# rmontanana/semcode

Measured on AMD Instinct MI355X. Metric: chunks/sec embed (256-tok) + top-k QPS over 10M x 768, higher is better.
Workload: dtype bf16; 1 GPU; encoder forward, 256 chunks x 256 tokens per GPU per step, BERT-base shape (12x768, 12 heads, FFN 3072), bf16 MFMA / f32 accumulate, random-init weights; global_batch=256, seq_len=256, parallelism=dp1 (replicated weights, no collective), device=AMD Radeon Graphics (gfx950:sramecc+:xnack-)

## Files before the change

### include/semcode_hip.h

```cpp
#ifndef SEMCODE_HIP_H
#define SEMCODE_HIP_H

#include <stddef.h>
#include <stdint.h>

#ifdef __cplusplus
extern "C" {
#endif

typedef int32_t sc_status;

enum {
    SC_OK = 0,
    SC_ERR_INVALID = -1,
    SC_ERR_HIP = -2,
    SC_ERR_STATE = -3,
    SC_ERR_UNSUPPORTED = -4,
    SC_ERR_NOMEM = -5
};

typedef enum { SC_METRIC_IP = 0, SC_METRIC_L2 = 1, SC_METRIC_COSINE = 2 } sc_metric;
typedef enum { SC_INDEX_FLAT = 0, SC_INDEX_IVF_FLAT = 1 } sc_index_kind;

typedef struct sc_runtime sc_runtime;
// ... 61 lines not shown
sc_status sc_tokenizer_create(const char* vocab_utf8, size_t nbytes, int32_t lowercase, sc_tokenizer** out);
sc_status sc_tokenizer_destroy(sc_tokenizer* tok);
sc_status sc_tokenizer_info(sc_tokenizer* tok, int32_t* vocab_size, int32_t* pad, int32_t* unk, int32_t* cls, int32_t* sep);
sc_status sc_tokenizer_encode(sc_tokenizer* tok, const char* bytes, const int64_t* offsets, int32_t n, int32_t max_tokens, int32_t S,
                              int32_t* ids, int32_t* lens, uint8_t* needs_fallback, int32_t threads);

sc_status sc_diag_gemm_bf16(sc_runtime* rt, int32_t epi, const float* A, const float* W, const float* bias, const float* R,
                            int32_t M, int32_t N, int32_t K, float* out);
sc_status sc_diag_gemm_bench(sc_runtime* rt, int32_t epi, int32_t M, int32_t N, int32_t K, int32_t iters, int32_t variant,
                             double* ms_per_launch);
sc_status sc_diag_gemm_trace(sc_runtime* rt, int32_t epi, int32_t M, int32_t N, int32_t K, uint64_t* out, int64_t cap_words);
sc_status sc_diag_gemm_i8(sc_runtime* rt, const int8_t* A, const int8_t* W, int32_t M, int32_t N, int32_t K, int32_t* out);
sc_status sc_diag_encoder_read(sc_encoder* enc, int32_t which, void* out, size_t nbytes);
sc_status sc_diag_set_option(const char* name, int32_t value);
sc_status sc_diag_rope(sc_runtime* rt, float* qk, int32_t rows, int32_t S, int32_t heads, float theta);
sc_status sc_diag_swiglu(sc_runtime* rt, const float* h, int32_t rows, int32_t F, float* out);
sc_status sc_diag_attention(sc_runtime* rt, const float* qkv, const int32_t* lens, int32_t B, int32_t S, int32_t heads, float* out);

sc_status sc_diag_fold_ln(sc_runtime* rt, const float* W, const float* gamma, const float* beta, const float* bias, int32_t N, int32_t K,
                          float* Wf, float* c1, float* c2);
sc_status sc_diag_gemm_lna(sc_runtime* rt, int32_t epi, int32_t flags, const float* A, const float* Wf, const float* c1, const float* c2,
                           const float* stats_in, float eps, int32_t M, int32_t N, int32_t K, int32_t rope_S, float rope_theta,
                           int32_t rope_ncols, float* C, float* fin);
sc_status sc_diag_gemm_resln(sc_runtime* rt, int32_t flags, const float* A, const float* W, const float* bias, const float* gam, const float* R,
                             const float* fin, float eps, int32_t M, int32_t N, int32_t K, float* C, float* stats_out);
sc_status sc_diag_attention_ex(sc_runtime* rt, const float* qkv, const int32_t* lens, int32_t B, int32_t S, int32_t heads, int32_t blocked_rows,
                               const float* slopes, float* out);
sc_status sc_diag_attention_packed(sc_runtime* rt, const float* qkv, const int32_t* starts, const int32_t* lens, int32_t B, int32_t heads,
                                   int32_t blocked_rows, const float* slopes, float* out);
sc_status sc_diag_layernorm(sc_runtime* rt, const float* x, int32_t tokens, int32_t H, const float* gamma, const float* beta, float eps, float* out);
sc_status sc_diag_mean_pool(sc_runtime* rt, const float* x, const int32_t* lens, int32_t B, int32_t S, int32_t H, int32_t normalize, float* out);
sc_status sc_diag_mean_pool_ln(sc_runtime* rt, const float* y, const float* stats, int32_t slots, int32_t tokens_pad, const float* gamma,
                               const float* beta, float eps, const int32_t* lens, int32_t B, int32_t S, int32_t H, float* out);
sc_status sc_diag_geglu(sc_runtime* rt, const float* h, int32_t rows, int32_t F, float* out);
sc_status sc_diag_embed(sc_runtime* rt, int32_t ln, const int32_t* ids, int32_t tokens, int32_t S, int32_t H, int32_t vocab, int32_t max_pos,
                        const float* wemb, const float* pemb, const float* temb, const float* gamma, const float* beta, float eps,
                        int32_t tokens_pad, int32_t slots, float* rows, float* stats);


sc_status sc_index_create(sc_runtime* rt, int32_t dim, sc_metric metric, sc_index_kind kind,
                          int32_t nlist, int64_t row_base, sc_index** out);
sc_status sc_index_destroy(sc_index* ix);
sc_status sc_index_info(sc_index* ix, int64_t* rows, int32_t* dim, int32_t* ld);
sc_status sc_index_reserve(sc_index* ix, int64_t rows);
sc_status sc_index_add(sc_index* ix, const float* vecs, int64_t n);
sc_status sc_index_overwrite(sc_index* ix, const float* vecs, const int64_t* rows, int64_t n);
// ... 80 lines not shown
```

### semcode_amd/_native.py

```python
from __future__ import annotations

import ctypes as C
import sys
import threading
from pathlib import Path

import numpy as np

LIB_PATH = Path(__file__).resolve().parent / "_lib" / "libsemcode_hip.so"

METRICS = {"IP": 0, "L2": 1, "COSINE": 2}
KINDS = {"FLAT": 0, "IVF_FLAT": 1}


class ScError(RuntimeError):

    def __init__(self, status: int, message: str):
        super().__init__(f"libsemcode_hip error {status}: {message}")
        self.status = status


class _Cfg(C.Structure):
    _fields_ = [("device", C.c_int32), ("stream", C.c_void_p), ("flags", C.c_int32)]

# ... 30 lines not shown
    "sc_encoder_embed_ids": (C.c_int32, [C.c_void_p, C.c_void_p, C.c_void_p, C.c_int32, C.c_int32, C.c_void_p]),
    "sc_encoder_embed_ids_dev": (C.c_int32, [C.c_void_p, C.c_void_p, C.c_void_p, C.c_int32, C.c_int32, C.c_void_p]),
    "sc_encoder_embed_ids_into": (C.c_int32, [C.c_void_p, C.c_void_p, C.c_void_p, C.c_int32, C.c_int32, C.c_void_p, C.c_void_p, C.c_void_p]),
    "sc_encoder_embed_ids_into_async": (C.c_int32, [C.c_void_p, C.c_void_p, C.c_void_p, C.c_int32, C.c_int32, C.c_void_p, C.c_void_p]),
    "sc_encoder_wait": (C.c_int32, [C.c_void_p]),
    "sc_encoder_packed_rows": (C.c_int32, [C.c_void_p, C.c_void_p, C.c_int32, C.POINTER(C.c_int64)]),
    "sc_encoder_embed_packed": (C.c_int32, [C.c_void_p, C.c_void_p, C.c_void_p, C.c_int32, C.c_void_p]),
    "sc_encoder_embed_packed_into": (C.c_int32, [C.c_void_p, C.c_void_p, C.c_void_p, C.c_int32, C.c_void_p, C.c_void_p, C.c_void_p]),
    "sc_encoder_embed_packed_into_async": (C.c_int32, [C.c_void_p, C.c_void_p, C.c_void_p, C.c_int32, C.c_void_p, C.c_void_p]),
    "sc_tokenizer_create": (C.c_int32, [C.c_char_p, C.c_size_t, C.c_int32, C.POINTER(C.c_void_p)]),
    "sc_tokenizer_destroy": (C.c_int32, [C.c_void_p]),
    "sc_tokenizer_info": (C.c_int32, [C.c_void_p] + [C.POINTER(C.c_int32)] * 5),
    "sc_tokenizer_encode": (C.c_int32, [C.c_void_p, C.c_char_p, C.c_void_p, C.c_int32, C.c_int32, C.c_int32, C.c_void_p, C.c_void_p, C.c_void_p, C.c_int32]),
    "sc_diag_gemm_bf16": (C.c_int32, [C.c_void_p, C.c_int32, C.c_void_p, C.c_void_p, C.c_void_p, C.c_void_p, C.c_int32, C.c_int32, C.c_int32, C.c_void_p]),
    "sc_diag_gemm_bench": (C.c_int32, [C.c_void_p, C.c_int32, C.c_int32, C.c_int32, C.c_int32, C.c_int32, C.c_int32, C.POINTER(C.c_double)]),
    "sc_diag_gemm_trace": (C.c_int32, [C.c_void_p, C.c_int32, C.c_int32, C.c_int32, C.c_int32, C.c_void_p, C.c_int64]),
    "sc_diag_set_option": (C.c_int32, [C.c_char_p, C.c_int32]),
    "sc_diag_gemm_i8": (C.c_int32, [C.c_void_p, C.c_void_p, C.c_void_p, C.c_int32, C.c_int32, C.c_int32, C.c_void_p]),
    "sc_diag_encoder_read": (C.c_int32, [C.c_void_p, C.c_int32, C.c_void_p, C.c_size_t]),
    "sc_diag_attention": (C.c_int32, [C.c_void_p, C.c_void_p, C.c_void_p, C.c_int32, C.c_int32, C.c_int32, C.c_void_p]),
    "sc_diag_rope": (C.c_int32, [C.c_void_p, C.c_void_p, C.c_int32, C.c_int32, C.c_int32, C.c_float]),
    "sc_diag_swiglu": (C.c_int32, [C.c_void_p, C.c_void_p, C.c_int32, C.c_int32, C.c_void_p]),
    "sc_diag_fold_ln": (C.c_int32, [C.c_void_p] * 5 + [C.c_int32, C.c_int32] + [C.c_void_p] * 3),
    "sc_diag_gemm_lna": (C.c_int32, [C.c_void_p, C.c_int32, C.c_int32] + [C.c_void_p] * 5 + [C.c_float, C.c_int32, C.c_int32, C.c_int32, C.c_int32,
                                     C.c_float, C.c_int32, C.c_void_p, C.c_void_p]),
    "sc_diag_gemm_resln": (C.c_int32, [C.c_void_p, C.c_int32] + [C.c_void_p] * 6 + [C.c_float, C.c_int32, C.c_int32, C.c_int32, C.c_void_p, C.c_void_p]),
    "sc_diag_attention_ex": (C.c_int32, [C.c_void_p, C.c_void_p, C.c_void_p, C.c_int32, C.c_int32, C.c_int32, C.c_int32, C.c_void_p, C.c_void_p]),
    "sc_diag_attention_packed": (C.c_int32, [C.c_void_p, C.c_void_p, C.c_void_p, C.c_void_p, C.c_int32, C.c_int32, C.c_int32, C.c_void_p, C.c_void_p]),
    "sc_diag_layernorm": (C.c_int32, [C.c_void_p, C.c_void_p, C.c_int32, C.c_int32, C.c_void_p, C.c_void_p, C.c_float, C.c_void_p]),
    "sc_diag_mean_pool": (C.c_int32, [C.c_void_p, C.c_void_p, C.c_void_p, C.c_int32, C.c_int32, C.c_int32, C.c_int32, C.c_void_p]),
    "sc_diag_mean_pool_ln": (C.c_int32, [C.c_void_p, C.c_void_p, C.c_void_p, C.c_int32, C.c_int32, C.c_void_p, C.c_void_p, C.c_float, C.c_void_p,
                                         C.c_int32, C.c_int32, C.c_int32, C.c_void_p]),
    "sc_diag_geglu": (C.c_int32, [C.c_void_p, C.c_void_p, C.c_int32, C.c_int32, C.c_void_p]),
    "sc_diag_embed": (C.c_int32, [C.c_void_p, C.c_int32, C.c_void_p, C.c_int32, C.c_int32, C.c_int32, C.c_int32, C.c_int32] + [C.c_void_p] * 5 +
                                 [C.c_float, C.c_int32, C.c_int32, C.c_void_p, C.c_void_p]),
    "sc_index_create": (C.c_int32, [C.c_void_p, C.c_int32, C.c_int32, C.c_int32, C.c_int32, C.c_int64, C.POINTER(C.c_void_p)]),
    "sc_index_destroy": (C.c_int32, [C.c_void_p]),
    "sc_index_info": (C.c_int32, [C.c_void_p, C.POINTER(C.c_int64), C.POINTER(C.c_int32), C.POINTER(C.c_int32)]),
    "sc_index_reserve": (C.c_int32, [C.c_void_p, C.c_int64]),
    "sc_index_add": (C.c_int32, [C.c_void_p, C.c_void_p, C.c_int64]),
    "sc_index_overwrite": (C.c_int32, [C.c_void_p, C.c_void_p, C.c_void_p, C.c_int64]),
    "sc_index_put_rows": (C.c_int32, [C.c_void_p, C.c_void_p, C.c_void_p, C.c_int64]),
    "sc_index_put_rows_dev": (C.c_int32, [C.c_void_p, C.c_void_p, C.c_void_p, C.c_int64]),
    "sc_index_delete_rows": (C.c_int32, [C.c_void_p, C.c_void_p, C.c_int64]),
    "sc_index_last_delete_stats": (C.c_int32, [C.c_void_p, C.POINTER(C.c_int64), C.POINTER(C.c_int64), C.POINTER(C.c_int32), C.POINTER(C.c_int32)]),
    "sc_index_get_rows": (C.c_int32, [C.c_void_p, C.c_int64, C.c_int64, C.c_void_p]),
# ... 736 lines not shown

def diag_fold_ln(rt: Runtime, W, gamma, beta, bias=None):
    W, gamma, beta = _f32(W), _f32(gamma), _f32(beta)
    bias = None if bias is None else _f32(bias)
    N, K = W.shape
    Wf, c1, c2 = np.empty((N, K), np.float32), np.empty(N, np.float32), np.empty(N, np.float32)
    _check(lib().sc_diag_fold_ln(rt.handle, _ptr(W), _ptr(gamma), _ptr(beta), _ptr(bias), N, K, _ptr(Wf), _ptr(c1), _ptr(c2)))
    return Wf, c1, c2


def diag_gemm_lna(rt: Runtime, epi: int, A, Wf, c1, c2, stats_in, eps: float, blocked: bool = False, rope_S: int = 0, rope_theta: float = 0.0,
                  rope_ncols: int = 0):
    A, Wf, c1, c2, stats_in = _f32(A), _f32(Wf), _f32(c1), _f32(c2), _f32(stats_in)
    M, K = A.shape
    N = Wf.shape[0]
    if stats_in.shape != (K // 256, M, 2) or Wf.shape != (N, K) or c1.shape != (N,) or c2.shape != (N,):
        raise ValueError("diag_gemm_lna: shapes")
    Cc, fin = np.empty((M, N), np.float32), np.empty((M, 2), np.float32)
    _check(lib().sc_diag_gemm_lna(rt.handle, epi, 1 if blocked else 0, _ptr(A), _ptr(Wf), _ptr(c1), _ptr(c2), _ptr(stats_in), float(eps), M, N, K,
                                  int(rope_S), float(rope_theta), int(rope_ncols), _ptr(Cc), _ptr(fin)))
    return (unblock64(Cc, M, N) if blocked else Cc), fin


def diag_gemm_resln(rt: Runtime, A, W, bias, gam, R, fin, eps: float, a_blocked: bool = False):
    A, W, bias, gam, R, fin = _f32(A), _f32(W), _f32(bias), _f32(gam), _f32(R), _f32(fin)
    M, K = A.shape
    N = W.shape[0]
    if W.shape != (N, K) or R.shape != (M, N) or fin.shape != (M, 2) or bias.shape != (N,) or gam.shape != (N,):
        raise ValueError("diag_gemm_resln: shapes")
    Ad = block64(A) if a_blocked else A
    Cc, st = np.empty((M, N), np.float32), np.empty((N // 256, M, 2), np.float32)
    _check(lib().sc_diag_gemm_resln(rt.handle, 1 if a_blocked else 0, _ptr(Ad), _ptr(W), _ptr(bias), _ptr(gam), _ptr(R), _ptr(fin), float(eps), M, N, K,
                                    _ptr(Cc), _ptr(st)))
    return Cc, st


def diag_attention_ex(rt: Runtime, qkv, lens, B: int, S: int, heads: int, blocked_rows: int = 0, slopes=None) -> np.ndarray:
    qkv = _f32(qkv)
    lens = np.ascontiguousarray(lens, np.int32)
    H = heads * 64
    if blocked_rows:
        pad = np.zeros((blocked_rows, 3 * H), np.float32)
        pad[: B * S] = qkv
        qkv = block64(pad)
    sl = None if slopes is None else _f32(slopes)
    out = np.empty((B * S, H), np.float32)
# ... 87 lines not shown
```

### semcode_amd/csrc/encoder_ops.h

```cpp
#pragma once
#include <vector>

#include "sc_common.h"

enum { EPI_BIAS = 0, EPI_BIAS_GELU = 1, EPI_BIAS_RES = 2, EPI_LNA_BIAS = 3, EPI_LNA_GELU = 4, EPI_RESLN_STATS = 5, EPI_LNA_BIAS_ROPE = 6 };

bool sc_gemm_bf16_supported(int M, int N, int K);
void sc_launch_gemm_bf16(int epi, const void* A, int lda, const void* W, int ldw, const float* bias, const void* R, int ldr, void* C,
                         int ldc, int M, int N, int K, hipStream_t s, void* splitk_scratch = nullptr, size_t splitk_scratch_bytes = 0);
int sc_gemm_splitk_factor(int M, int N, int K, int cus);
bool sc_gemm_ln_supported(int M, int N, int K);
void sc_launch_gemm_bf16_ln(int epi, const void* A, int lda, const void* W, int ldw, const float* bias, const void* R, int ldr, void* C, int ldc, int M,
                            int N, int K, hipStream_t s, const float* c1, const float* stats_in, float* fin, const float* gam, float* stats_out, float eps,
                            const float* rope_cos = nullptr, const float* rope_sin = nullptr, int rope_S = 0, int rope_ncols = 0);
void sc_launch_gemm_i8_diag(const void* A, const void* W, void* C, int M, int N, int K, hipStream_t s);
void sc_gemm_set_debug(int v);
void sc_gemm_set_order(int v);
void sc_gemm_set_pp(int v);
void sc_gemm_set_nt(int v);
void sc_gemm_set_trace(unsigned long long* dev);
void sc_gemm_force_tile128(bool on);

void sc_launch_embed_ln(const int32_t* ids, int tokens, int S, int H, int vocab, int max_pos, const float* wemb, const float* pemb,
                        const float* temb, const float* g, const float* b, float eps, void* out, hipStream_t s);
void sc_launch_layernorm(const void* in, int tokens, int H, const float* g, const float* b, float eps, void* out, hipStream_t s);
bool sc_attention_supported(int S, int H, int heads);
void sc_launch_attention(const void* qkv, const int32_t* lens, int B, int S, int H, const float* slopes, void* ctx, hipStream_t s, int blocked = 0);
void sc_launch_geglu(const void* h, int64_t tokens, int F, void* out, hipStream_t s);
void sc_launch_swiglu(const void* h, int64_t tokens, int F, void* out, hipStream_t s);
void sc_launch_rope_qk(void* qkv, int64_t M, int nblocks, int S, const float* cos_t, const float* sin_t, hipStream_t s);
void sc_launch_embed_raw(const int32_t* ids, int tokens, int tokens_pad, int S, int H, int vocab, int max_pos, const float* wemb, const float* pemb,
                         const float* temb, void* out, float* stats, int slots, hipStream_t s);
void sc_launch_fold_ln_weights(const float* W, const float* gamma, const float* beta, const float* bias, int N, int K, void* Wf, float* c1, float* c2,
                               hipStream_t s);
void sc_launch_add_vectors(const float* a, const float* b, float* out, int n, hipStream_t s);
void sc_launch_mean_pool_ln(const void* y, const float* stats, int slots, int tokens_pad, const float* gamma, const float* beta, float eps,
                            const int32_t* lens, int B, int S, int H, float* out, hipStream_t s);
void sc_launch_mean_pool(const void* x, const int32_t* lens, int B, int S, int H, int normalize, float* out, hipStream_t s);
void sc_launch_f32_to_bf16(const float* in, void* out, int64_t n, hipStream_t s);
void sc_launch_synth_scaled(float* out, int64_t n, uint64_t seed, float scale, float offset, hipStream_t s);
void sc_launch_bf16_to_f32(const void* in, float* out, int64_t n, hipStream_t s);

// ... 16 lines not shown
```

### semcode_amd/csrc/gemm_bf16.hip

```cpp
#include <algorithm>
#include <cstdlib>

#include "encoder_ops.h"
#include "gemm_tile.h"

#ifndef SC_GEMM_PP_DEFAULT
#define SC_GEMM_PP_DEFAULT 4
#endif


struct GemmArgs {
    const bf16_t* A;
    const bf16_t* W;
    const float* bias;
    const bf16_t* R;
    bf16_t* C;
    int M, N, K, lda, ldw, ldr, ldc;
    int tiles_n;
    int ntiles;
    int order;
    int splitk;
    float* partial;
    unsigned long long* trace;
    int nt;
    int cblock;
    int ablock;
    const float* c1;
    const float* stats_in;
    int stat_slots;
    float* fin;
    const float* gam;
    float* stats_out;
    float ln_eps;
    const float* rope_cos;
    const float* rope_sin;
    int rope_smask, rope_ncols;
};

static __device__ __forceinline__ size_t c_index(const GemmArgs& a, int64_t m, int n) {
    return a.cblock ? ((size_t)(n >> 6) * (size_t)a.M + (size_t)m) * 64 + (size_t)(n & 63) : (size_t)m * a.ldc + n;
}

template <int EPI>
__global__ __launch_bounds__(256) void gemm_bf16_kernel(GemmArgs a) {
// ... 182 lines not shown
        for (int ni = 0; ni < 4; ++ni) {
            f32x4 v = acc[ni][mi] + bias4[ni];
            if (EPI == EPI_BIAS_GELU) {
                const f32x2 g0 = gelu_erf_fast2(f32x2{v[0], v[1]}), g1 = gelu_erf_fast2(f32x2{v[2], v[3]});
                v = f32x4{g0[0], g0[1], g1[0], g1[1]};
            }
            if (EPI == EPI_BIAS_RES) {
                const u32x2 r2 = rr[mi][ni];
                v += f32x4{__builtin_bit_cast(float, r2[0] << 16), __builtin_bit_cast(float, r2[0] & 0xFFFF0000u),
                           __builtin_bit_cast(float, r2[1] << 16), __builtin_bit_cast(float, r2[1] & 0xFFFF0000u)};
            }
            *reinterpret_cast<u32x2*>(stg + fr * T_EPI_ROW + (ni * 16 + 4 * fq) * 2) = u32x2{pack_bf16x2(v[0], v[1]), pack_bf16x2(v[2], v[3])};
        }
#pragma unroll
        for (int j = 0; j < 2; ++j) {
            const u32x4 o = *reinterpret_cast<const u32x4*>(stg + (j * 8 + prow) * T_EPI_ROW + c8 * 2);
            bf16_t* dst = cp + (size_t)(mi * 16 + j * 8) * crs;
            if (a.nt) asm volatile("global_store_dwordx4 %0, %1, off nt" ::"v"(dst), "v"(o) : "memory");
            else *reinterpret_cast<u32x4*>(dst) = o;
        }
    }
}

template <int EPI>
static __device__ __forceinline__ void gemm256_epilogue_lna(const GemmArgs& a, int m0, int n0, char* smem, int w, int lane, f32x4 (&acc)[4][8]) {
    const int wm = w >> 2, wn = w & 3;
    int ln = lane;
    asm volatile("" : "+v"(ln));
    __builtin_amdgcn_sched_barrier(0);
    const int fr = ln & 15, fq = ln >> 4;
    const int prow = ln >> 3, c8 = (ln & 7) * 8;
    char* stg = smem + 4 * T_TILE_BYTES + w * (16 * T_EPI_ROW);
    typedef uint32_t u32x2 __attribute__((ext_vector_type(2)));
    typedef uint32_t u32x4 __attribute__((ext_vector_type(4)));
    typedef float f32x2_t __attribute__((ext_vector_type(2)));
    f32x4 c1v[4], c2v[4];
#pragma unroll
    for (int ni = 0; ni < 4; ++ni) {
        c1v[ni] = *reinterpret_cast<const f32x4*>(a.c1 + n0 + wn * 64 + ni * 16 + 4 * fq);
        c2v[ni] = *reinterpret_cast<const f32x4*>(a.bias + n0 + wn * 64 + ni * 16 + 4 * fq);
    }
    asm volatile("s_waitcnt vmcnt(0)" ::: "memory");
    char* slice = smem + w * 16384;
    {
        f32x4 sacc = {0.f, 0.f, 0.f, 0.f};
        for (int t = 0; t < a.stat_slots; ++t) sacc += *reinterpret_cast<const f32x4*>(slice + t * 1024 + ln * 16);
        const float inv_k = 1.0f / (float)a.K;
        const float mu0 = sacc[0] * inv_k, mu1 = sacc[2] * inv_k;
        const float rs0 = __builtin_amdgcn_rsqf(fmaxf(fmaf(-mu0, mu0, sacc[1] * inv_k), 0.f) + a.ln_eps);
        const float rs1 = __builtin_amdgcn_rsqf(fmaxf(fmaf(-mu1, mu1, sacc[3] * inv_k), 0.f) + a.ln_eps);
        const f32x4 fin4 = {mu0, rs0, mu1, rs1};
        *reinterpret_cast<f32x4*>(slice + ln * 16) = fin4;
        if (n0 == 0 && wn == 0) *reinterpret_cast<f32x4*>(a.fin + (size_t)(m0 + wm * 128) * 2 + ln * 4) = fin4;
    }
    const char* sl = slice + fr * 8;
    const size_t crs = a.cblock ? 64 : (size_t)a.ldc;
    bf16_t* cp = a.C + c_index(a, m0 + wm * 128 + prow, n0 + wn * 64) + c8;
#pragma unroll
    for (int mi = 0; mi < 8; ++mi) {
        const f32x2_t st = *reinterpret_cast<const f32x2_t*>(sl + mi * 128);
        const float mu = st[0], rs = st[1];
        f32x2 nrm = {-rs * mu, -rs * mu}, rs2 = {rs, rs};
        SC_OPAQUE_PAIR(nrm);
        SC_OPAQUE_PAIR(rs2);
#pragma unroll
        for (int ni = 0; ni < (EPI == EPI_LNA_BIAS_ROPE ? 0 : 4); ++ni) {
            const f32x2 d01 = __builtin_elementwise_fma(nrm, f32x2{c1v[ni][0], c1v[ni][1]}, f32x2{c2v[ni][0], c2v[ni][1]});
            const f32x2 d23 = __builtin_elementwise_fma(nrm, f32x2{c1v[ni][2], c1v[ni][3]}, f32x2{c2v[ni][2], c2v[ni][3]});
            const f32x2 v01 = __builtin_elementwise_fma(rs2, f32x2{acc[ni][mi][0], acc[ni][mi][1]}, d01);
            const f32x2 v23 = __builtin_elementwise_fma(rs2, f32x2{acc[ni][mi][2], acc[ni][mi][3]}, d23);
            f32x4 v = {v01[0], v01[1], v23[0], v23[1]};
            if (EPI == EPI_LNA_GELU) {
                const f32x2 g0 = gelu_erf_fast2(f32x2{v[0], v[1]}), g1 = gelu_erf_fast2(f32x2{v[2], v[3]});
                v = f32x4{g0[0], g0[1], g1[0], g1[1]};
            }
            *reinterpret_cast<u32x2*>(stg + fr * T_EPI_ROW + (ni * 16 + 4 * fq) * 2) = u32x2{pack_bf16x2(v[0], v[1]), pack_bf16x2(v[2], v[3])};
        }
        if constexpr (EPI == EPI_LNA_BIAS_ROPE) {
// ... 170 lines not shown
                                         ResLnCoopHook{ResidualCoopHook{a.R + (size_t)m0 * a.ldr + n0, a.ldr, w, lane, smem},
                                                       a.fin + (size_t)(m0 + (w >> 2) * 128) * 2}, a_kstep);
        else
            gemm256_mainloop_sel<PP, ML>(a, lda, m0, n0, smem, acc, w, lane,
                                         ResLnTailHook{ResidualTailHook{a.R + (size_t)m0 * a.ldr + n0, a.ldr, w, lane, smem},
                                                       a.fin + (size_t)(m0 + (w >> 2) * 128) * 2}, a_kstep);
    }
    else if (EPI == EPI_LNA_BIAS || EPI == EPI_LNA_GELU || EPI == EPI_LNA_BIAS_ROPE)
        gemm256_mainloop_sel<PP, ML>(a, lda, m0, n0, smem, acc, w, lane,
                                     LnaTailHook{a.stats_in + (size_t)(m0 + (w >> 2) * 128) * 2, (size_t)a.M * 2, a.stat_slots, w, lane, smem}, a_kstep);
    else
        gemm256_mainloop_sel<PP, ML>(a, lda, m0, n0, smem, acc, w, lane, NoTailHook{}, a_kstep);
    gemm256_stamp(a, blockIdx.x, 3);
    if (DBG & 4) {
        float sink = 0.f;
#pragma unroll
        for (int i = 0; i < 4; ++i)
#pragma unroll
            for (int j = 0; j < 8; ++j) sink += acc[i][j][0] + acc[i][j][3];
        if (sink == 12345.678f) a.C[0] = 1;
        return;
    }
    if (EPI == EPI_RESLN_STATS) gemm256_epilogue_resln<COOP>(a, m0, n0, smem, w, lane, acc);
    else if (EPI == EPI_LNA_BIAS || EPI == EPI_LNA_GELU || EPI == EPI_LNA_BIAS_ROPE) gemm256_epilogue_lna<EPI>(a, m0, n0, smem, w, lane, acc);
    else gemm256_epilogue<EPI, COOP && !(DBG & 31)>(a, m0, n0, smem, w, lane, acc);
    if (a.trace) {
        gemm256_stamp(a, blockIdx.x, 4);
        asm volatile("s_waitcnt vmcnt(0)" ::: "memory");
        gemm256_stamp(a, blockIdx.x, 5);
    }
}

__global__ __launch_bounds__(512) void gemm256_i8_diag_kernel(const int8_t* __restrict__ A, const int8_t* __restrict__ W, int32_t* __restrict__ C, int M, int N,
                                                               int K) {
    extern __shared__ __attribute__((aligned(16))) char smem[];
    const int lane = threadIdx.x & 63;
    const int w = __builtin_amdgcn_readfirstlane(threadIdx.x >> 6);
    const int tiles_n = N / T_BN;
    const int m0 = ((int)blockIdx.x / tiles_n) * T_BM, n0 = ((int)blockIdx.x % tiles_n) * T_BN;
    f32x4 acc[4][8];
#pragma unroll
    for (int i = 0; i < 4; ++i)
#pragma unroll
        for (int j = 0; j < 8; ++j) acc[i][j] = f32x4{0.f, 0.f, 0.f, 0.f};
    gemm_tile256_mainloop<0, NoTailHook, true>(reinterpret_cast<const bf16_t*>(A), K / 2, m0, reinterpret_cast<const bf16_t*>(W), K / 2, n0, K / 2, smem, acc, w, lane);
    int ln = lane;
    asm volatile("" : "+v"(ln));
    const int wm = w >> 2, wn = w & 3, fr = ln & 15, fq = ln >> 4;
    int32_t* out = C + (size_t)(m0 + wm * 128 + fr) * N + n0 + wn * 64 + 4 * fq;
#pragma unroll
    for (int mi = 0; mi < 8; ++mi)
#pragma unroll
// ... 62 lines not shown
    }
}

int sc_gemm_splitk_factor(int M, int N, int K, int cus) {
    if ((M % T_BM) || (N % T_BN) || M > 1024) return 1;
    const int tiles = (M / T_BM) * (N / T_BN), nk = K / G_BK;
    int best = 1;
    for (int d = 2; d <= nk; ++d)
        if (nk % d == 0 && nk / d >= 3 && tiles * d <= cus) best = d;
    return tiles * 2 <= cus ? best : 1;
}

static int g_gemm_pp = -1;
void sc_gemm_set_pp(int v) { g_gemm_pp = v; }
static int gemm_pp() {
    static const char* env = getenv("SC_GEMM_PP");
    return g_gemm_pp >= 0 ? g_gemm_pp : env ? atoi(env) : SC_GEMM_PP_DEFAULT;
}
static int g_gemm_nt = -1;
void sc_gemm_set_nt(int v) { g_gemm_nt = v < 0 ? -1 : (v ? 1 : 0); }
static int gemm_nt(int M, int N) {
    static const char* env_nt = getenv("SC_GEMM_NT");
    return g_gemm_nt >= 0 ? g_gemm_nt : env_nt ? atoi(env_nt) : ((size_t)M * (size_t)N * 2 >= ((size_t)64 << 20));
}
template <int EPI, int DBG, int PP>
static void launch256_pp(const GemmArgs& a, dim3 grid, dim3 block, hipStream_t s) {
    static ScDeviceOnce once;
    sc_device_once(once, [&] { hipFuncSetAttribute(reinterpret_cast<const void*>(gemm256_bf16_kernel<EPI, DBG, PP>), hipFuncAttributeMaxDynamicSharedMemorySize, (int)T_LDS_BYTES); });
    hipLaunchKernelGGL((gemm256_bf16_kernel<EPI, DBG, PP>), grid, block, T_LDS_BYTES, s, a);
}
template <int EPI, int DBG>
static void launch256(const GemmArgs& a, dim3 grid, dim3 block, hipStream_t s) {
    const int pp = a.K >= 2 * G_BK ? gemm_pp() : 0;
    if (pp == 0) return launch256_pp<EPI, DBG, 0>(a, grid, block, s);
    if constexpr (DBG == 4) {
        if (pp == 3) return launch256_pp<EPI, DBG, 3>(a, grid, block, s);
        if (pp == 5) return launch256_pp<EPI, DBG, 5>(a, grid, block, s);
    }
    launch256_pp<EPI, DBG, 4>(a, grid, block, s);
}
template <int DBG>
static void launch256_epi(int epi, const GemmArgs& a, dim3 grid, dim3 block, hipStream_t s) {
    if (epi == EPI_BIAS_GELU) launch256<EPI_BIAS_GELU, DBG>(a, grid, block, s);
    else if (epi == EPI_BIAS_RES) launch256<EPI_BIAS_RES, DBG>(a, grid, block, s);
    else launch256<EPI_BIAS, DBG>(a, grid, block, s);
}

bool sc_gemm_ln_supported(int M, int N, int K) { return M > 0 && (M % T_BM) == 0 && (N % T_BN) == 0 && (K % 256) == 0; }
void sc_launch_gemm_bf16_ln(int epi, const void* A, int lda, const void* W, int ldw, const float* bias, const void* R, int ldr, void* C, int ldc, int M,
                            int N, int K, hipStream_t s, const float* c1, const float* stats_in, float* fin, const float* gam, float* stats_out, float eps,
                            const float* rope_cos, const float* rope_sin, int rope_S, int rope_ncols) {
    GemmArgs a;
    a.rope_cos = rope_cos; a.rope_sin = rope_sin; a.rope_smask = rope_S - 1; a.rope_ncols = rope_ncols;
    a.A = (const bf16_t*)A; a.W = (const bf16_t*)W; a.bias = bias; a.R = (const bf16_t*)R; a.C = (bf16_t*)C;
    a.M = M; a.N = N; a.K = K; a.lda = lda; a.ldw = ldw; a.ldr = ldr; a.ldc = ldc;
    a.cblock = ldc == SC_LDC_BLOCKED64 ? 1 : 0;
    a.ablock = lda == SC_LDC_BLOCKED64 ? 1 : 0;
    static const char* env_order = getenv("SC_GEMM_ORDER");
    a.order = env_order ? atoi(env_order) : ((size_t)N * (size_t)K * 2 <= ((size_t)8 << 20) ? 0 : 16);
    a.trace = nullptr;
    a.nt = gemm_nt(M, N);
    a.tiles_n = N / T_BN;
    a.ntiles = (M / T_BM) * a.tiles_n;
    a.splitk = 1;
    a.partial = nullptr;
    a.c1 = c1; a.stats_in = stats_in; a.stat_slots = K / 256; a.fin = fin; a.gam = gam; a.stats_out = stats_out; a.ln_eps = eps;
    dim3 grid((unsigned)a.ntiles), block(512);
    if (epi == EPI_LNA_BIAS) launch256<EPI_LNA_BIAS, 0>(a, grid, block, s);
    else if (epi == EPI_LNA_BIAS_ROPE) launch256<EPI_LNA_BIAS_ROPE, 0>(a, grid, block, s);
    else if (epi == EPI_LNA_GELU) launch256<EPI_LNA_GELU, 0>(a, grid, block, s);
    else launch256<EPI_RESLN_STATS, 0>(a, grid, block, s);
}

void sc_launch_gemm_bf16(int epi, const void* A, int lda, const void* W, int ldw, const float* bias, const void* R, int ldr, void* C,
                         int ldc, int M, int N, int K, hipStream_t s, void* splitk_scratch, size_t splitk_scratch_bytes) {
    GemmArgs a;
    a.c1 = nullptr; a.stats_in = nullptr; a.stat_slots = 0; a.fin = nullptr; a.gam = nullptr; a.stats_out = nullptr; a.ln_eps = 0.f;
    a.rope_cos = nullptr; a.rope_sin = nullptr; a.rope_smask = 0; a.rope_ncols = 0;
    a.A = (const bf16_t*)A; a.W = (const bf16_t*)W; a.bias = bias; a.R = (const bf16_t*)R; a.C = (bf16_t*)C;
    a.M = M; a.N = N; a.K = K; a.lda = lda; a.ldw = ldw; a.ldr = ldr; a.ldc = ldc;
    a.cblock = ldc == SC_LDC_BLOCKED64 ? 1 : 0;
    a.ablock = lda == SC_LDC_BLOCKED64 ? 1 : 0;
    static const char* env_order = getenv("SC_GEMM_ORDER");
    a.order = env_order ? atoi(env_order) : g_gemm_order >= 0 ? g_gemm_order : ((size_t)N * (size_t)K * 2 <= ((size_t)8 << 20) ? 0 : 16);
    a.trace = g_gemm_trace;
    a.nt = gemm_nt(M, N);
    if ((M % T_BM) == 0 && (N % T_BN) == 0 && !g_force_tile128) {
        a.tiles_n = N / T_BN;
        a.ntiles = (M / T_BM) * a.tiles_n;
        dim3 grid((unsigned)a.ntiles), block(512);
        a.splitk = 1;
        a.partial = nullptr;
        if (splitk_scratch && !g_gemm_dbg && !g_gemm_trace) {
            const int d = sc_gemm_splitk_factor(M, N, K, sc_device_cus());
            if (d > 1 && (size_t)d * M * N * sizeof(float) <= splitk_scratch_bytes) {
                a.splitk = d;
                a.partial = (float*)splitk_scratch;
                static ScDeviceOnce once_sk;
                sc_device_once(once_sk, [&] { hipFuncSetAttribute(reinterpret_cast<const void*>(gemm256_splitk_kernel), hipFuncAttributeMaxDynamicSharedMemorySize, (int)T_LDS_BYTES); });
                hipLaunchKernelGGL(gemm256_splitk_kernel, dim3((unsigned)(a.ntiles * d)), block, T_LDS_BYTES, s, a);
                const int rb = (int)std::min<int64_t>(((int64_t)M * (N / 4) + 255) / 256, 1024);
                if (epi == EPI_BIAS_GELU) hipLaunchKernelGGL(gemm_splitk_reduce_kernel<EPI_BIAS_GELU>, dim3((unsigned)rb), dim3(256), 0, s, a);
                else if (epi == EPI_BIAS_RES) hipLaunchKernelGGL(gemm_splitk_reduce_kernel<EPI_BIAS_RES>, dim3((unsigned)rb), dim3(256), 0, s, a);
                else hipLaunchKernelGGL(gemm_splitk_reduce_kernel<EPI_BIAS>, dim3((unsigned)rb), dim3(256), 0, s, a);
                return;
            }
        }
        switch (g_gemm_dbg) {
            case 1: launch256<EPI_BIAS, 1>(a, grid, block, s); return;
            case 2: launch256<EPI_BIAS, 2>(a, grid, block, s); return;
            case 4: launch256<EPI_BIAS, 4>(a, grid, block, s); return;
            case 5: launch256<EPI_BIAS, 5>(a, grid, block, s); return;
            case 20: launch256<EPI_BIAS, 20>(a, grid, block, s); return;
            case 21: launch256<EPI_BIAS, 21>(a, grid, block, s); return;
// ... 20 lines not shown
```

### semcode_amd/csrc/sc_api.cpp

```cpp
#include <algorithm>
#include <cmath>
#include <cstdarg>
#include <cstdio>
#include <cstring>
#include <mutex>
#include <new>
#include <string>
#include <vector>

#include "encoder_ops.h"
#include "sc_internal.h"

static thread_local std::string g_err;

sc_status sc_fail(sc_status code, const char* fmt, ...) {
    char buf[512];
    va_list ap;
    va_start(ap, fmt);
    vsnprintf(buf, sizeof buf, fmt, ap);
    va_end(ap);
    g_err = buf;
    return code;
}

// ... 141 lines not shown
}

extern "C" sc_status sc_synth_fill_dev(sc_runtime* rt, float* out, int64_t rows, int32_t dim, int32_t ld, uint64_t seed,
                                       int64_t first_row) {
    if (!rt || !out) return sc_fail(SC_ERR_INVALID, "sc_synth_fill_dev: NULL argument");
    if (rows < 0 || dim <= 0 || ld < dim || (ld & 3)) return sc_fail(SC_ERR_INVALID, "sc_synth_fill_dev: need rows>=0, 0<dim<=ld, ld%%4==0");
    SC_HIP(hipSetDevice(rt->device));
    sc_launch_synth_fill(out, rows, dim, ld, seed, first_row, nullptr, rt->stream);
    SC_HIP(hipGetLastError());
    return SC_OK;
}

extern "C" sc_status sc_diag_set_option(const char* name, int32_t value) {
    if (!name) return sc_fail(SC_ERR_INVALID, "sc_diag_set_option: NULL name");
    static const struct { const char* name; void (*set)(int); } options[] = {
        {"coarse_workgroups", sc_scan_set_coarse_workgroups}, {"coarse_persistent", sc_scan_set_coarse_persistent},
        {"gemm_pp", sc_gemm_set_pp},                          {"gemm_nt", sc_gemm_set_nt},
        {"ivf_refresh_nomem", sc_ivf_set_refresh_nomem},      {"ivf_refine_cap", sc_ivf_set_refine_cap},
        {"ivf_coarse_nomem", sc_ivf_set_coarse_nomem},        {"collect_pass", sc_set_collect_pass},
        {"tighten", sc_set_tighten},                          {"wide_candidates", sc_set_wide_force},
        {"ivf_tail_rows", sc_set_ivf_tail_rows},              {"delete_chunk_rows", sc_set_delete_chunk_rows},
        {"rope_fused", sc_encoder_set_rope_fused},            {"mask_gather", sc_set_mask_gather},
        {"group_width0", sc_set_group_width0},                {"group_width1", sc_set_group_width1},
        {"mmr_chunk_q", sc_set_mmr_chunk_q},
    };
    for (const auto& o : options)
        if (!strcmp(name, o.name)) {
            o.set(value);
            return SC_OK;
        }
    return sc_fail(SC_ERR_INVALID, "sc_diag_set_option: unknown option '%s'", name);
}


static inline int round_up(int v, int a) { return (v + a - 1) / a * a; }

extern "C" sc_status sc_index_create(sc_runtime* rt, int32_t dim, sc_metric metric, sc_index_kind kind, int32_t nlist,
                                     int64_t row_base, sc_index** out) {
    if (!rt || !out) return sc_fail(SC_ERR_INVALID, "sc_index_create: NULL argument");
    *out = nullptr;
    if (dim <= 0 || dim > 65536) return sc_fail(SC_ERR_INVALID, "sc_index_create: dim %d out of range", dim);
    if (metric != SC_METRIC_IP && metric != SC_METRIC_L2 && metric != SC_METRIC_COSINE)
        return sc_fail(SC_ERR_INVALID, "sc_index_create: unknown metric %d", (int)metric);
    if (kind != SC_INDEX_FLAT && kind != SC_INDEX_IVF_FLAT) return sc_fail(SC_ERR_INVALID, "sc_index_create: unknown kind %d", (int)kind);
    if (kind == SC_INDEX_IVF_FLAT && nlist < 1) return sc_fail(SC_ERR_INVALID, "sc_index_create: IVF_FLAT needs nlist >= 1");
    sc_index* ix = new (std::nothrow) sc_index();
    if (!ix) return sc_fail(SC_ERR_NOMEM, "out of host memory");
// ... 390 lines not shown
```

### semcode_amd/csrc/sc_encoder_diag.cpp

```cpp
#include <cstring>
#include <vector>

#include "encoder_ops.h"
#include "sc_internal.h"

namespace {
#define SC_TRY(expr)              \
    do {                          \
        sc_status st_ = (expr);   \
        if (st_) return st_;      \
    } while (0)

sc_status dev_alloc(sc_devbuf& out, size_t bytes) {
    if (out.alloc(bytes) != hipSuccess) return sc_fail(SC_ERR_NOMEM, "diag: hipMalloc failed");
    return SC_OK;
}
sc_status upload(const void* host, size_t bytes, sc_devbuf& out, hipStream_t s) {
    SC_TRY(dev_alloc(out, bytes));
    if (host && bytes) SC_HIP(hipMemcpyAsync(out.p, host, bytes, hipMemcpyHostToDevice, s));
    return SC_OK;
}
sc_status upload_bf16(const float* host, int64_t n, sc_devbuf& f32buf, sc_devbuf& out, hipStream_t s) {
    SC_TRY(upload(host, (size_t)n * 4, f32buf, s));
    SC_TRY(dev_alloc(out, (size_t)n * 2));
// ... 182 lines not shown
    hipStream_t s = rt->stream;
    sc_devbuf fa, da, fw, dw, dc1, dc2, dst, dfin, dc, dt;
    SC_TRY(upload_bf16(A, (int64_t)M * K, fa, da, s));
    SC_TRY(upload_bf16(Wf, (int64_t)N * K, fw, dw, s));
    SC_TRY(upload(c1, (size_t)N * 4, dc1, s));
    SC_TRY(upload(c2, (size_t)N * 4, dc2, s));
    SC_TRY(upload(stats_in, (size_t)(K / 256) * M * 8, dst, s));
    SC_TRY(alloc_nan(dfin, (size_t)M * 8, s));
    SC_TRY(alloc_nan(dc, (size_t)M * N * 2, s));
    const float *cos_t = nullptr, *sin_t = nullptr;
    std::vector<float> tab;
    if (rope) {
        tab = sc_rope_table(rope_S, rope_theta);
        SC_TRY(upload(tab.data(), tab.size() * 4, dt, s));
        cos_t = (const float*)dt.p;
        sin_t = cos_t + tab.size() / 2;
    }
    sc_launch_gemm_bf16_ln(epi, da.p, K, dw.p, K, (const float*)dc2.p, nullptr, 0, dc.p, (flags & 1) ? SC_LDC_BLOCKED64 : N, M, N, K, s, (const float*)dc1.p,
                           (const float*)dst.p, (float*)dfin.p, nullptr, nullptr, eps, cos_t, sin_t, rope ? rope_S : 0, rope ? rope_ncols : 0);
    SC_TRY(download(dfin.p, (size_t)M * 8, fin, s));
    return download_bf16(dc.p, (int64_t)M * N, C, s);
}

extern "C" sc_status sc_diag_gemm_resln(sc_runtime* rt, int32_t flags, const float* A, const float* W, const float* bias, const float* gam, const float* R,
                                        const float* fin, float eps, int32_t M, int32_t N, int32_t K, float* C, float* stats_out) {
    if (!rt || !A || !W || !bias || !gam || !R || !fin || !C || !stats_out) return sc_fail(SC_ERR_INVALID, "sc_diag_gemm_resln: NULL argument");
    if ((flags & ~1) || !(eps > 0.f)) return sc_fail(SC_ERR_INVALID, "sc_diag_gemm_resln: bad flags / eps");
    if (!sc_gemm_ln_supported(M, N, K)) return sc_fail(SC_ERR_UNSUPPORTED, "sc_diag_gemm_resln: need M%%256==0, N%%256==0, K%%256==0");
    SC_HIP(hipSetDevice(rt->device));
    hipStream_t s = rt->stream;
    sc_devbuf fa, da, fw, dw, fr, dr, db, dg, dfin, dc, dso;
    SC_TRY(upload_bf16(A, (int64_t)M * K, fa, da, s));
    SC_TRY(upload_bf16(W, (int64_t)N * K, fw, dw, s));
    SC_TRY(upload_bf16(R, (int64_t)M * N, fr, dr, s));
    SC_TRY(upload(bias, (size_t)N * 4, db, s));
    SC_TRY(upload(gam, (size_t)N * 4, dg, s));
    SC_TRY(upload(fin, (size_t)M * 8, dfin, s));
    SC_TRY(alloc_nan(dc, (size_t)M * N * 2, s));
    SC_TRY(alloc_nan(dso, (size_t)(N / 256) * M * 8, s));
    sc_launch_gemm_bf16_ln(EPI_RESLN_STATS, da.p, (flags & 1) ? SC_LDC_BLOCKED64 : K, dw.p, K, (const float*)db.p, dr.p, N, dc.p, N, M, N, K, s, nullptr, nullptr,
                           (float*)dfin.p, (const float*)dg.p, (float*)dso.p, eps);
    SC_TRY(download(dso.p, (size_t)(N / 256) * M * 8, stats_out, s));
    return download_bf16(dc.p, (int64_t)M * N, C, s);
}

static sc_status diag_attention(const char* who, sc_runtime* rt, const float* qkv, const int32_t* lens, int32_t B, int32_t S, int32_t heads, int32_t blocked_rows,
// ... 161 lines not shown
```

Before: 22350 chunks/s.

## Add persistent strip kernel for LN-fused GEMMs reusing A panel across N tiles

Adds a strip kernel for the LayerNorm-folded GEMM epilogues (QKV and FFN-up). Each workgroup keeps one 256-row A panel and walks a contiguous strip of N tiles. It finalises the LN row statistics once per strip instead of once per tile, and uses a hook to prefetch the next tile's weights during the current mainloop. A rule turns the strip path on by default for K=768 with 9 or 12 N tiles when the strip count balances across CUs. The cost is fewer, longer workgroups, which can hurt load balance and latency hiding. It also needs an extra 8 KB of LDS per block.

```diff
diff --git a/include/semcode_hip.h b/include/semcode_hip.h
--- a/include/semcode_hip.h
+++ b/include/semcode_hip.h
@@ -107,6 +107,7 @@
 sc_status sc_diag_gemm_lna(sc_runtime* rt, int32_t epi, int32_t flags, const float* A, const float* Wf, const float* c1, const float* c2,
                            const float* stats_in, float eps, int32_t M, int32_t N, int32_t K, int32_t rope_S, float rope_theta,
                            int32_t rope_ncols, float* C, float* fin);
+int32_t sc_diag_gemm_strip(int32_t M, int32_t N, int32_t K, int32_t cus);
 sc_status sc_diag_gemm_resln(sc_runtime* rt, int32_t flags, const float* A, const float* W, const float* bias, const float* gam, const float* R,
                              const float* fin, float eps, int32_t M, int32_t N, int32_t K, float* C, float* stats_out);
 sc_status sc_diag_attention_ex(sc_runtime* rt, const float* qkv, const int32_t* lens, int32_t B, int32_t S, int32_t heads, int32_t blocked_rows,
diff --git a/semcode_amd/_native.py b/semcode_amd/_native.py
--- a/semcode_amd/_native.py
+++ b/semcode_amd/_native.py
@@ -76,6 +76,7 @@
     "sc_diag_rope": (C.c_int32, [C.c_void_p, C.c_void_p, C.c_int32, C.c_int32, C.c_int32, C.c_float]),
     "sc_diag_swiglu": (C.c_int32, [C.c_void_p, C.c_void_p, C.c_int32, C.c_int32, C.c_void_p]),
     "sc_diag_fold_ln": (C.c_int32, [C.c_void_p] * 5 + [C.c_int32, C.c_int32] + [C.c_void_p] * 3),
+    "sc_diag_gemm_strip": (C.c_int32, [C.c_int32] * 4),
     "sc_diag_gemm_lna": (C.c_int32, [C.c_void_p, C.c_int32, C.c_int32] + [C.c_void_p] * 5 + [C.c_float, C.c_int32, C.c_int32, C.c_int32, C.c_int32,
                                      C.c_float, C.c_int32, C.c_void_p, C.c_void_p]),
     "sc_diag_gemm_resln": (C.c_int32, [C.c_void_p, C.c_int32] + [C.c_void_p] * 6 + [C.c_float, C.c_int32, C.c_int32, C.c_int32, C.c_void_p, C.c_void_p]),
@@ -858,6 +859,10 @@
     return (unblock64(Cc, M, N) if blocked else Cc), fin
 
 
+def diag_gemm_strip(M: int = 0, N: int = 0, K: int = 0, cus: int = 0) -> int:
+    return int(lib().sc_diag_gemm_strip(int(M), int(N), int(K), int(cus)))
+
+
 def diag_gemm_resln(rt: Runtime, A, W, bias, gam, R, fin, eps: float, a_blocked: bool = False):
     A, W, bias, gam, R, fin = _f32(A), _f32(W), _f32(bias), _f32(gam), _f32(R), _f32(fin)
     M, K = A.shape
diff --git a/semcode_amd/csrc/encoder_ops.h b/semcode_amd/csrc/encoder_ops.h
--- a/semcode_amd/csrc/encoder_ops.h
+++ b/semcode_amd/csrc/encoder_ops.h
@@ -18,6 +18,11 @@
 void sc_gemm_set_order(int v);
 void sc_gemm_set_pp(int v);
 void sc_gemm_set_nt(int v);
+void sc_gemm_set_strip(int v);
+void sc_gemm_set_strip_n(int v);
+int sc_gemm_strip_rule(int M, int N, int K, int cus);
+int sc_gemm_strip_tiles(int M, int N, int K, int cus, bool a_blocked = false);
+int sc_gemm_last_strip(void);
 void sc_gemm_set_trace(unsigned long long* dev);
 void sc_gemm_force_tile128(bool on);
 
diff --git a/semcode_amd/csrc/gemm_bf16.hip b/semcode_amd/csrc/gemm_bf16.hip
--- a/semcode_amd/csrc/gemm_bf16.hip
+++ b/semcode_amd/csrc/gemm_bf16.hip
@@ -20,6 +20,7 @@
     int ntiles;
     int order;
     int splitk;
+    int strip;
     float* partial;
     unsigned long long* trace;
     int nt;
@@ -248,8 +249,16 @@
     }
 }
 
-template <int EPI>
-static __device__ __forceinline__ void gemm256_epilogue_lna(const GemmArgs& a, int m0, int n0, char* smem, int w, int lane, f32x4 (&acc)[4][8]) {
+static __device__ __forceinline__ f32x4 lna_finalise(const GemmArgs& a, const f32x4& sacc) {
+    const float inv_k = 1.0f / (float)a.K;
+    const float mu0 = sacc[0] * inv_k, mu1 = sacc[2] * inv_k;
+    const float rs0 = __builtin_amdgcn_rsqf(fmaxf(fmaf(-mu0, mu0, sacc[1] * inv_k), 0.f) + a.ln_eps);
+    const float rs1 = __builtin_amdgcn_rsqf(fmaxf(fmaf(-mu1, mu1, sacc[3] * inv_k), 0.f) + a.ln_eps);
+    return f32x4{mu0, rs0, mu1, rs1};
+}
+
+template <int EPI, bool STRIP = false>
+static __device__ __forceinline__ void gemm256_epilogue_lna(const GemmArgs& a, int m0, int n0, char* smem, int w, int lane, f32x4 (&acc)[4][8], char* mrs) {
     const int wm = w >> 2, wn = w & 3;
     int ln = lane;
     asm volatile("" : "+v"(ln));
@@ -266,20 +275,15 @@
         c1v[ni] = *reinterpret_cast<const f32x4*>(a.c1 + n0 + wn * 64 + ni * 16 + 4 * fq);
         c2v[ni] = *reinterpret_cast<const f32x4*>(a.bias + n0 + wn * 64 + ni * 16 + 4 * fq);
     }
-    asm volatile("s_waitcnt vmcnt(0)" ::: "memory");
-    char* slice = smem + w * 16384;
-    {
+    if constexpr (!STRIP) {
+        asm volatile("s_waitcnt vmcnt(0)" ::: "memory");
         f32x4 sacc = {0.f, 0.f, 0.f, 0.f};
-        for (int t = 0; t < a.stat_slots; ++t) sacc += *reinterpret_cast<const f32x4*>(slice + t * 1024 + ln * 16);
-        const float inv_k = 1.0f / (float)a.K;
-        const float mu0 = sacc[0] * inv_k, mu1 = sacc[2] * inv_k;
-        const float rs0 = __builtin_amdgcn_rsqf(fmaxf(fmaf(-mu0, mu0, sacc[1] * inv_k), 0.f) + a.ln_eps);
-        const float rs1 = __builtin_amdgcn_rsqf(fmaxf(fmaf(-mu1, mu1, sacc[3] * inv_k), 0.f) + a.ln_eps);
-        const f32x4 fin4 = {mu0, rs0, mu1, rs1};
-        *reinterpret_cast<f32x4*>(slice + ln * 16) = fin4;
+        for (int t = 0; t < a.stat_slots; ++t) sacc += *reinterpret_cast<const f32x4*>(mrs + t * 1024 + ln * 16);
+        const f32x4 fin4 = lna_finalise(a, sacc);
+        *reinterpret_cast<f32x4*>(mrs + ln * 16) = fin4;
         if (n0 == 0 && wn == 0) *reinterpret_cast<f32x4*>(a.fin + (size_t)(m0 + wm * 128) * 2 + ln * 4) = fin4;
     }
-    const char* sl = slice + fr * 8;
+    const char* sl = mrs + fr * 8;
     const size_t crs = a.cblock ? 64 : (size_t)a.ldc;
     bf16_t* cp = a.C + c_index(a, m0 + wm * 128 + prow, n0 + wn * 64) + c8;
 #pragma unroll
@@ -496,12 +500,66 @@
         return;
     }
     if (EPI == EPI_RESLN_STATS) gemm256_epilogue_resln<COOP>(a, m0, n0, smem, w, lane, acc);
-    else if (EPI == EPI_LNA_BIAS || EPI == EPI_LNA_GELU || EPI == EPI_LNA_BIAS_ROPE) gemm256_epilogue_lna<EPI>(a, m0, n0, smem, w, lane, acc);
+    else if (EPI == EPI_LNA_BIAS || EPI == EPI_LNA_GELU || EPI == EPI_LNA_BIAS_ROPE) gemm256_epilogue_lna<EPI>(a, m0, n0, smem, w, lane, acc, smem + w * 16384);
     else gemm256_epilogue<EPI, COOP && !(DBG & 31)>(a, m0, n0, smem, w, lane, acc);
     if (a.trace) {
         gemm256_stamp(a, blockIdx.x, 4);
         asm volatile("s_waitcnt vmcnt(0)" ::: "memory");
         gemm256_stamp(a, blockIdx.x, 5);
+    }
+}
+
+#define T_STRIP_LDS_BYTES (T_LDS_BYTES + 8 * 1024)
+template <int EPI, int PP>
+__global__ __launch_bounds__(512) void gemm256_strip_kernel(GemmArgs a) {
+    extern __shared__ __attribute__((aligned(16))) char smem[];
+    const int lane = threadIdx.x & 63;
+    const int w = __builtin_amdgcn_readfirstlane(threadIdx.x >> 6);
+    const int spp = (a.tiles_n + a.strip - 1) / a.strip;
+    const int sid = xcd_remap(blockIdx.x, gridDim.x);
+    const int mt = sid / spp;
+    const int m0 = __builtin_amdgcn_readfirstlane(mt * T_BM);
+    const int t0 = __builtin_amdgcn_readfirstlane((sid - mt * spp) * a.strip);
+    const int t1 = t0 + a.strip < a.tiles_n ? t0 + a.strip : a.tiles_n;
+    char* mrs = smem + T_LDS_BYTES + w * 1024;
+    {
+        int ln = lane;
+        asm volatile("" : "+v"(ln));
+        const float* st = a.stats_in + (size_t)(m0 + (w >> 2) * 128) * 2 + ln * 4;
+        f32x4 sacc = {0.f, 0.f, 0.f, 0.f};
+        for (int t = 0; t < a.stat_slots; ++t) sacc += *reinterpret_cast<const f32x4*>(st + (size_t)t * a.M * 2);
+        const f32x4 fin4 = lna_finalise(a, sacc);
+        *reinterpret_cast<f32x4*>(mrs + ln * 16) = fin4;
+        if (t0 == 0 && (w & 3) == 0) *reinterpret_cast<f32x4*>(a.fin + (size_t)(m0 + (w >> 2) * 128) * 2 + ln * 4) = fin4;
+    }
+    const int lda = a.lda;
+    const size_t a_kstep = G_BK;
+    PPNextTileHook hook;
+    hook.a_kbytes = (uint32_t)(G_BK * 2); hook.a1_off = (uint32_t)(64 * lda * 2); hook.w1_off = (uint32_t)(32 * a.ldw * 2);
+    hook.w = w; hook.smem = smem;
+    hook.ra = __builtin_amdgcn_make_buffer_rsrc((void*)(a.A + (size_t)m0 * lda), 0, -1, 0x00020000);
+#pragma unroll 1
+    for (int t = t0; t < t1; ++t) {
+        const int n0 = __builtin_amdgcn_readfirstlane(t * T_BN);
+        const bool first = t == t0, last = t + 1 == t1;
+        int ln = lane;
+        asm volatile("" : "+v"(ln));
+        hook.rw = __builtin_amdgcn_make_buffer_rsrc((void*)(a.W + (size_t)(last ? n0 : n0 + T_BN) * a.ldw), 0, -1, 0x00020000);
+        f32x4 acc[4][8];
+#pragma unroll
+        for (int i = 0; i < 4; ++i)
+#pragma unroll
+            for (int j = 0; j < 8; ++j) acc[i][j] = f32x4{0.f, 0.f, 0.f, 0.f};
+        if (first) {
+            if (last) gemm_tile256_mainloop_pp<PP, 0, NoTailHook, false, false>(a.A, lda, m0, a.W, a.ldw, n0, a.K, smem, acc, w, ln, NoTailHook{}, a_kstep);
+            else gemm_tile256_mainloop_pp<PP, 0, PPNextTileHook, false, false>(a.A, lda, m0, a.W, a.ldw, n0, a.K, smem, acc, w, ln, hook, a_kstep);
+        } else {
+            if (last) gemm_tile256_mainloop_pp<PP, 0, NoTailHook, false, true>(a.A, lda, m0, a.W, a.ldw, n0, a.K, smem, acc, w, ln, NoTailHook{}, a_kstep);
+            else gemm_tile256_mainloop_pp<PP, 0, PPNextTileHook, false, true>(a.A, lda, m0, a.W, a.ldw, n0, a.K, smem, acc, w, ln, hook, a_kstep);
+        }
+        asm volatile("" ::: "memory");
+        __builtin_amdgcn_sched_barrier(0);
+        gemm256_epilogue_lna<EPI, true>(a, m0, n0, smem, w, lane, acc, mrs);
     }
 }
 
@@ -610,6 +668,34 @@
 static int gemm_nt(int M, int N) {
     static const char* env_nt = getenv("SC_GEMM_NT");
     return g_gemm_nt >= 0 ? g_gemm_nt : env_nt ? atoi(env_nt) : ((size_t)M * (size_t)N * 2 >= ((size_t)64 << 20));
+}
+static int g_gemm_strip = -1, g_gemm_strip_n = 0, g_gemm_strip_last = 0;
+void sc_gemm_set_strip(int v) { g_gemm_strip = v < 0 ? -1 : v; }
+void sc_gemm_set_strip_n(int v) { g_gemm_strip_n = v > 0 ? v : 0; }
+int sc_gemm_last_strip(void) { return g_gemm_strip_last; }
+int sc_gemm_strip_rule(int M, int N, int K, int cus) {
+    if (M <= 0 || (M % T_BM) || N <= 0 || (N % T_BN) || K != 768 || cus <= 0) return 0;
+    const int tiles_n = N / T_BN, L = tiles_n == 9 ? 3 : tiles_n == 12 ? 6 : 0;
+    if (!L) return 0;
+    const int64_t panels = M / T_BM, strips = panels * (tiles_n / L), tiles = panels * tiles_n;
+    if (strips < (int64_t)cus) return 0;
+    return ((strips + cus - 1) / cus) * L <= (tiles + cus - 1) / cus ? L : 0;
+}
+int sc_gemm_strip_tiles(int M, int N, int K, int cus, bool a_blocked) {
+    static const char* env = getenv("SC_GEMM_STRIP");
+    if (K < 256 || gemm_pp() == 0 || a_blocked || g_gemm_trace || g_gemm_dbg) return 0;
+    int v = g_gemm_strip >= 0 ? g_gemm_strip : env ? atoi(env) : -1;
+    if (v >= 0 && g_gemm_strip_n && N != g_gemm_strip_n) v = 0;
+    if (v < 0) v = sc_gemm_strip_rule(M, N, K, cus);
+    return std::min(v, N / T_BN);
+}
+template <int EPI>
+static void launch256_strip(GemmArgs a, int strip, hipStream_t s) {
+    static ScDeviceOnce once;
+    sc_device_once(once, [&] { hipFuncSetAttribute(reinterpret_cast<const void*>(gemm256_strip_kernel<EPI, 4>), hipFuncAttributeMaxDynamicSharedMemorySize, (int)T_STRIP_LDS_BYTES); });
+    a.strip = strip;
+    const unsigned grid = (unsigned)((a.M / T_BM) * ((a.tiles_n + strip - 1) / strip));
+    hipLaunchKernelGGL((gemm256_strip_kernel<EPI, 4>), dim3(grid), dim3(512), T_STRIP_LDS_BYTES, s, a);
 }
 template <int EPI, int DBG, int PP>
 static void launch256_pp(const GemmArgs& a, dim3 grid, dim3 block, hipStream_t s) {
@@ -654,6 +740,16 @@
     a.partial = nullptr;
     a.c1 = c1; a.stats_in = stats_in; a.stat_slots = K / 256; a.fin = fin; a.gam = gam; a.stats_out = stats_out; a.ln_eps = eps;
     dim3 grid((unsigned)a.ntiles), block(512);
+    a.strip = 0;
+    if (epi != EPI_RESLN_STATS) {
+        g_gemm_strip_last = sc_gemm_strip_tiles(M, N, K, sc_device_cus(), a.ablock != 0);
+        if (const int strip = g_gemm_strip_last) {
+            if (epi == EPI_LNA_BIAS) launch256_strip<EPI_LNA_BIAS>(a, strip, s);
+            else if (epi == EPI_LNA_BIAS_ROPE) launch256_strip<EPI_LNA_BIAS_ROPE>(a, strip, s);
+            else launch256_strip<EPI_LNA_GELU>(a, strip, s);
+            return;
+        }
+    }
     if (epi == EPI_LNA_BIAS) launch256<EPI_LNA_BIAS, 0>(a, grid, block, s);
     else if (epi == EPI_LNA_BIAS_ROPE) launch256<EPI_LNA_BIAS_ROPE, 0>(a, grid, block, s);
     else if (epi == EPI_LNA_GELU) launch256<EPI_LNA_GELU, 0>(a, grid, block, s);
@@ -678,6 +774,7 @@
         a.ntiles = (M / T_BM) * a.tiles_n;
         dim3 grid((unsigned)a.ntiles), block(512);
         a.splitk = 1;
+        a.strip = 0;
         a.partial = nullptr;
         if (splitk_scratch && !g_gemm_dbg && !g_gemm_trace) {
             const int d = sc_gemm_splitk_factor(M, N, K, sc_device_cus());
diff --git a/semcode_amd/csrc/sc_api.cpp b/semcode_amd/csrc/sc_api.cpp
--- a/semcode_amd/csrc/sc_api.cpp
+++ b/semcode_amd/csrc/sc_api.cpp
@@ -187,7 +187,8 @@
         {"ivf_tail_rows", sc_set_ivf_tail_rows},              {"delete_chunk_rows", sc_set_delete_chunk_rows},
         {"rope_fused", sc_encoder_set_rope_fused},            {"mask_gather", sc_set_mask_gather},
         {"group_width0", sc_set_group_width0},                {"group_width1", sc_set_group_width1},
-        {"mmr_chunk_q", sc_set_mmr_chunk_q},
+        {"mmr_chunk_q", sc_set_mmr_chunk_q},                  {"gemm_strip", sc_gemm_set_strip},
+        {"gemm_strip_n", sc_gemm_set_strip_n},
     };
     for (const auto& o : options)
         if (!strcmp(name, o.name)) {
diff --git a/semcode_amd/csrc/sc_encoder_diag.cpp b/semcode_amd/csrc/sc_encoder_diag.cpp
--- a/semcode_amd/csrc/sc_encoder_diag.cpp
+++ b/semcode_amd/csrc/sc_encoder_diag.cpp
@@ -228,6 +228,11 @@
     return download_bf16(dc.p, (int64_t)M * N, C, s);
 }
 
+extern "C" int32_t sc_diag_gemm_strip(int32_t M, int32_t N, int32_t K, int32_t cus) {
+    if (M == 0) return sc_gemm_last_strip();
+    return sc_gemm_strip_tiles(M, N, K, cus > 0 ? cus : sc_device_cus());
+}
+
 extern "C" sc_status sc_diag_gemm_resln(sc_runtime* rt, int32_t flags, const float* A, const float* W, const float* bias, const float* gam, const float* R,
                                         const float* fin, float eps, int32_t M, int32_t N, int32_t K, float* C, float* stats_out) {
     if (!rt || !A || !W || !bias || !gam || !R || !fin || !C || !stats_out) return sc_fail(SC_ERR_INVALID, "sc_diag_gemm_resln: NULL argument");
```

Measured after the change: 23050 chunks/s (median of 6 runs). 1.03x the previous value.
